# TankMermaid/GraphAligner

Measured on AMD Instinct MI355X. Metric: aligned Gbp/sec (whole node), 10kb ONT reads vs chr-scale GFA, higher is better.
Workload: dtype u64

## Files before the change

graphaligner_amd/csrc/ga_device.hip:

```cpp
#include <hip/hip_runtime.h>

#include <algorithm>
#include <cstdio>
#include <cstdlib>
#include <cstring>
#include <memory>
#include <mutex>
#include <vector>

#include "../../include/graphaligner_amd.h"
#include "ga_backend.h"
#include "ga_kernel.h"
#include "ga_lanes.h"
#include "ga_seed_dev.h"

namespace {

#define HIP_OK(call) do { hipError_t e_ = (call); if (e_ != hipSuccess) { fprintf(stderr, "graphaligner_amd: %s failed: %s\n", #call, hipGetErrorString(e_)); return GA_E_DEVICE; } } while (0)

struct SlotLayout
{
	uint64_t endPrev, endCur, sliceOff, arena, trace, flags, ckpt, belowOff, sparse, ovr, bytes;
};
__host__ __device__ inline SlotLayout slotLayout(uint32_t capCols, uint32_t maxSlices, uint64_t arenaWords, uint32_t traceCap, uint32_t sparseBw = 0)
{
	auto up = [](uint64_t x) { return (x + 255) & ~255ull; };
	SlotLayout l;
	uint64_t at = 0;
	l.endPrev = at; at = up(at + 4ull * capCols);
	l.endCur = at; at = up(at + 4ull * capCols);
	l.sliceOff = at; at = up(at + 4ull * (maxSlices + 1));
	l.arena = at; at = up(at + 4ull * arenaWords);
	l.trace = at; at = up(at + 1ull * traceCap + 64);
	l.flags = at; at = up(at + maxSlices + 1);
	l.ckpt = at; at = up(at + 4ull * (maxSlices + 2));
	l.belowOff = at; at = up(at + 4ull * (maxSlices + 1));
	l.sparse = at; if (sparseBw) at = up(at + gak::sparse_mem_bytes(sparseBw));
	l.ovr = at; if (sparseBw) at = up(at + 8ull * (maxSlices + 2));
	l.bytes = at;
	return l;
}

#ifndef GA_WAVES_EU
#define GA_WAVES_EU 4
#endif
template <int MAXN, bool GENERAL, bool SPARSE = false>
__global__ void __launch_bounds__(64) __attribute__((amdgpu_waves_per_eu(GA_WAVES_EU, 8))) ga_extend_kernel(GaLaunch L)
{
	__shared__ gak::WaveState<MAXN> ws;
	const SlotLayout lay = slotLayout(L.cap_cols, L.max_slices, L.arena_words, L.trace_cap, SPARSE ? L.sparse_bw : 0u);
	uint8_t* base = L.scratch + (uint64_t)blockIdx.x * L.slot_bytes;
	gak::Slot slot;
	slot.end_prev = (uint32_t*)(base + lay.endPrev);
	slot.end_cur = (uint32_t*)(base + lay.endCur);
	slot.slice_off = (uint32_t*)(base + lay.sliceOff);
	slot.arena = (uint32_t*)(base + lay.arena);
	slot.trace = base + lay.trace;
	slot.slice_flags = base + lay.flags;
	slot.ckpt = (uint32_t*)(base + lay.ckpt);
	slot.below_off = (uint32_t*)(base + lay.belowOff);
	slot.sparse = SPARSE ? base + lay.sparse : nullptr;
	slot.ovr = SPARSE ? (uint32_t*)(base + lay.ovr) : nullptr;
	slot.sparse_max_bw = SPARSE ? L.sparse_bw : 0u;
	while (true)
	{
		uint32_t k = gaw::wave_atomic_add(L.next_job, 1u);
		if (k >= L.n_jobs) break;
		uint32_t job = L.job_list ? L.job_list[k] : k;
		gak::run_job<MAXN, GENERAL, SPARSE>(L, ws, slot, job);
		__syncthreads();
	}
}

template <int N, int LW>
__global__ void __launch_bounds__(64) __attribute__((amdgpu_waves_per_eu(1, 2))) ga_lanes_kernel(gal::GaLanesLaunch L)
{
	using namespace gal;
	__shared__ uint32_t lds[Lay<N>::WORDS * LW + LW * kStageWords64 * 2 + 128];
	const int lane = (int)threadIdx.x;
	const WaveLayout lay = wave_layout<N>(L.cap_cols, L.cap_rows, L.max_slices, L.cap_moves, LW);
	uint8_t* base = L.scratch + (uint64_t)blockIdx.x * L.wave_bytes;
	while (true)
	{
		const uint32_t grp = gaw::wave_atomic_add(L.next_group, 1u);
		const uint64_t first = (uint64_t)grp * L.lanes_per_wave;
		if (first >= L.n_jobs) break;
		const bool hasJob = lane < (int)L.lanes_per_wave && lane < LW && first + (uint32_t)lane < L.n_jobs;
		const uint32_t jobIndex = hasJob ? (L.job_list ? L.job_list[first + (uint32_t)lane] : (uint32_t)(first + (uint32_t)lane)) : 0u;
		LaneMem m;
		m.lane = lane < LW ? lane : 0;
		m.tid = lane;
		m.flushPart = (uint32_t)lane % 12u; m.flushLane = (uint32_t)lane / 12u;
		m.ls = LW;
		m.lds.base = lds + (lane < LW ? lane : 0);
		m.lds.lw = LW;
		m.stage = (uint64_t*)(lds + Lay<N>::WORDS * LW);
		m.laneBlocks = lds + Lay<N>::WORDS * LW + LW * kStageWords64 * 2;
		m.usedChunks = 12u * (L.lanes_per_wave < (uint32_t)LW ? L.lanes_per_wave : (uint32_t)LW);
		m.endPrev = (uint32_t*)(base + lay.endA) + m.lane;
		m.endCur = (uint32_t*)(base + lay.endB) + m.lane;
		m.hdr = (uint32_t*)(base + lay.hdr) + m.lane;
		m.snodes = (uint32_t*)(base + lay.snodes) + m.lane;
		m.moves = (uint32_t*)(base + lay.moves) + m.lane;
		m.arena = base + lay.arena;
		LaneState st;
#if GA_STAMPS == 3
		const uint64_t wall0 = wall_clock64(), cyc0 = gaw::stamp();
#endif
		uint64_t tA = gaw::stamp(), tB, acc[4] = {0, 0, 0, 0};
#define GAL_LAP(i) do { tB = gaw::stamp(); acc[i] += tB - tA; tA = tB; } while (0)
		lane_begin<N>(L, m, st, jobIndex, hasJob);
		uint32_t blockTop = 0;
		for (uint32_t slice = 0; ; slice++)
		{
			lane_band<N>(L, m, st, slice);
			GAL_LAP(0);
			if (!__ballot(st.live)) break;
			fill_slice<N, 8, LW>(L.graph, m, st, slice, st.live, blockTop, L.cap_rows, L.cap_cols);
			GAL_LAP(1);
			lane_end_slice<N>(L, m, st, slice);
			GAL_LAP(2);
		}
		lane_finish<N>(L, m, st, hasJob);
		GAL_LAP(3);
#undef GAL_LAP
#ifdef GA_STAMPS
		if (hasJob && lane == 0) { GaJobOut* o = L.outs + st.job; o->stamps[1] = acc[0]; o->stamps[4] = acc[1]; o->stamps[0] = acc[2]; o->stamps[5] = acc[3]; o->stamps[2] = st.laps[0]; o->stamps[3] = st.laps[1]; o->stamps[6] = st.laps[2]; o->stamps[7] = st.laps[7];
#if GA_STAMPS == 4
			o->stamps[6] = acc[0]; o->stamps[7] = acc[1];
			for (int i = 0; i < 5; i++) o->stamps[i] = st.blaps[i];
#endif
#if GA_STAMPS == 3
			o->stamps[0] = wall0; o->stamps[1] = wall_clock64(); o->stamps[4] = gaw::stamp() - cyc0;
#endif
#if GA_STAMPS == 2
			o->stamps[0] = st.laps[4]; o->stamps[1] = st.laps[5]; o->stamps[4] = st.laps[6];
#endif
		}
#endif
		__syncthreads();
	}
}

__global__ void __launch_bounds__(64) ga_eq_words_kernel(const uint8_t* __restrict__ seq, const GaEqFill* __restrict__ fills, uint32_t nFills, const uint8_t* __restrict__ lut,
                                                         uint32_t padCode, uint64_t* __restrict__ eq, uint8_t* __restrict__ flags, uint8_t* __restrict__ rows)
{
	__shared__ uint8_t t[512];
	const uint32_t lane = threadIdx.x;
	for (uint32_t i = lane; i < 512; i += 64) t[i] = lut[i];
	__syncthreads();
	for (uint32_t fi = blockIdx.x; fi < nFills; fi += gridDim.x)
	{
		const GaEqFill f = fills[fi];
		const uint8_t* s = seq + f.seq_off;
		bool bad = false;
		for (uint32_t r0 = 0; r0 < f.padded; r0 += 64)
		{
			const uint32_t k = r0 + lane;
			uint32_t code = padCode;
			if (k < f.n) code = f.backward ? t[256 + s[f.n - 1 - k]] : t[s[f.pos + k]];
			rows[f.eq_slice * 64 + k] = (uint8_t)code;
			const uint64_t e0 = __ballot(code & 1u), e1 = __ballot(code & 2u), e2 = __ballot(code & 4u), e3 = __ballot(code & 8u);
			const uint64_t inv = __ballot(code & GA_ROW_INVALID);
			const uint32_t last = (uint32_t)__builtin_amdgcn_readlane((int)code, 63);
			const uint64_t meta = (uint64_t)((last >> 4) & 7u) | (inv ? 8u : 0u);
			if (lane < 5) eq[(f.eq_slice + r0 / 64) * 5 + lane] = lane == 0 ? e0 : lane == 1 ? e1 : lane == 2 ? e2 : lane == 3 ? e3 : meta;
			bad = bad || inv != 0;
		}
		if (lane == 0) flags[fi] = bad ? 1 : 0;
	}
}

__global__ void ga_outs_init_kernel(GaJobOut* outs, uint32_t n)
{
	const uint32_t i = blockIdx.x * blockDim.x + threadIdx.x;
	if (i >= n) return;
	GaJobOut o;
	memset(&o, 0, sizeof(o));
	o.status = GA_NOT_RUN;
	outs[i] = o;
}

struct PinnedPool
{
	std::mutex lock;
	std::vector<std::pair<size_t, char*>> idle;
	~PinnedPool() { for (auto& b : idle) hipHostFree(b.second); }
};

struct DevGraph : GaBackendGraph
{
	std::shared_ptr<PinnedPool> pinned = std::make_shared<PinnedPool>();
	bool buildsMatchWords() const override { return true; }
	std::shared_ptr<char> hostBlock(size_t bytes) override
	{
		const size_t two = (size_t)2 << 20;
		bytes = (bytes + two - 1) & ~(two - 1);
		std::shared_ptr<PinnedPool> pool = pinned;
		char* p = nullptr;
		size_t cap = 0;
		{
			std::lock_guard<std::mutex> guard(pool->lock);
			size_t best = pool->idle.size();
			for (size_t i = 0; i < pool->idle.size(); i++)
				if (pool->idle[i].first >= bytes && pool->idle[i].first <= 2 * bytes + two && (best == pool->idle.size() || pool->idle[i].first < pool->idle[best].first)) best = i;
			if (best != pool->idle.size()) { cap = pool->idle[best].first; p = pool->idle[best].second; pool->idle.erase(pool->idle.begin() + (long)best); }
		}
		if (!p)
		{
			hipSetDevice(device);
			if (hipHostMalloc((void**)&p, bytes, hipHostMallocDefault) != hipSuccess) return GaBackendGraph::hostBlock(bytes);
			cap = bytes;
		}
		return std::shared_ptr<char>(p, [pool, cap](char* q) {
			std::lock_guard<std::mutex> guard(pool->lock);
			if (pool->idle.size() < 6) pool->idle.emplace_back(cap, q); else hipHostFree(q);
		});
	}

	std::unique_ptr<gasd::DevSeedEngine> seed;
	GaSeedEngine* seedEngine() override { return seed.get(); }

	int device = 0;
	GaDevGraph g;
	GaHmmTables* hmm = nullptr;
	std::vector<void*> allocs;
	int cus = 0;
	uint64_t totalBp = 0;
	uint8_t* pool = nullptr;
	size_t poolBytes = 0;
	bool poolBusy = false;
	~DevGraph() override
	{
		hipSetDevice(device);
		for (void* p : allocs) hipFree(p);
		for (auto& b : idleBlocks) hipFree(b.second);
		if (pool) hipFree(pool);
		if (hostPool) hipHostFree(hostPool);
	}
	std::mutex blockLock;
	std::vector<std::pair<size_t, void*>> idleBlocks;
	void* takeBlock(size_t bytes)
	{
		{
			std::lock_guard<std::mutex> lock(blockLock);
			size_t best = idleBlocks.size();
			for (size_t i = 0; i < idleBlocks.size(); i++)
				if (idleBlocks[i].first >= bytes && idleBlocks[i].first <= bytes + bytes / 2 + 4096 && (best == idleBlocks.size() || idleBlocks[i].first < idleBlocks[best].first)) best = i;
			if (best != idleBlocks.size())
			{
				void* p = idleBlocks[best].second;
				idleBlocks.erase(idleBlocks.begin() + (long)best);
				return p;
			}
		}
		void* p = nullptr;
		if (hipMalloc(&p, bytes) != hipSuccess) return nullptr;
		return p;
	}
	void giveBlock(void* p, size_t bytes)
	{
		std::lock_guard<std::mutex> lock(blockLock);
		if (idleBlocks.size() >= 48) { hipFree(idleBlocks.front().second); idleBlocks.erase(idleBlocks.begin()); }
		idleBlocks.emplace_back(bytes, p);
	}
	std::mutex poolLock;
	uint8_t* takePool(size_t bytes)
	{
		std::lock_guard<std::mutex> lock(poolLock);
		if (poolBusy) return nullptr;
		if (bytes > poolBytes)
		{
			if (pool) hipFree(pool);
			pool = nullptr; poolBytes = 0;
			if (hipMalloc((void**)&pool, bytes) != hipSuccess) { pool = nullptr; return nullptr; }
			poolBytes = bytes;
		}
		poolBusy = true;
		return pool;
	}
	void givePool() { std::lock_guard<std::mutex> lock(poolLock); poolBusy = false; }
	size_t poolBytesIfFree() { std::lock_guard<std::mutex> lock(poolLock); return poolBusy ? 0 : poolBytes; }
	std::mutex hostLock;
	uint8_t* hostPool = nullptr;
	size_t hostPoolBytes = 0;
	bool hostPoolBusy = false;
	uint8_t* takeHost(size_t bytes)
	{
		std::lock_guard<std::mutex> lock(hostLock);
		if (hostPoolBusy) return nullptr;
		if (bytes > hostPoolBytes)
		{
			if (hostPool) hipHostFree(hostPool);
			hostPool = nullptr; hostPoolBytes = 0;
			const size_t want = bytes + bytes / 8;
			if (hipHostMalloc((void**)&hostPool, want, hipHostMallocDefault) != hipSuccess) { hostPool = nullptr; return nullptr; }
			hostPoolBytes = want;
		}
		hostPoolBusy = true;
		return hostPool;
	}
	void giveHost() { std::lock_guard<std::mutex> lock(hostLock); hostPoolBusy = false; }
	template <typename T> int put(const std::vector<T>& v, const T** out)
	{
		void* p = nullptr;
		HIP_OK(hipMalloc(&p, std::max<size_t>(v.size() * sizeof(T), 16)));
		allocs.push_back(p);
		HIP_OK(hipMemcpy(p, v.data(), v.size() * sizeof(T), hipMemcpyHostToDevice));
		*out = (const T*)p;
		return 0;
	}
};

struct Knobs
{
	int lanes = -1;
	int spread = 1;
	bool debugPasses = false;
	uint64_t tracePoolBytes = 0;
	Knobs()
	{
		if (const char* e = getenv("GA_LANES")) lanes = atoi(e) != 0 ? 1 : 0;
		debugPasses = getenv("GA_DEBUG_PASSES") != nullptr;
		if (const char* e = getenv("GA_LANES_SPREAD")) spread = atoi(e);
		if (const char* t = getenv("GA_TEST_TRACE_POOL_BYTES")) tracePoolBytes = (uint64_t)atoll(t) & ~3ull;
	}
};

struct DevBatch : GaBackendBatch
{
	DevGraph* g = nullptr;
	Knobs knobs;
	hipStream_t stream = nullptr;
	hipEvent_t evA = nullptr, evB = nullptr;
	std::vector<std::pair<size_t, void*>> allocs;
	std::vector<GaJob> jobs;
	GaRunConfig cfg;
	GaLaunch L;
	const uint64_t* dEq = nullptr;
	uint32_t* dList = nullptr;
	size_t dListCap = 0;
	std::vector<GaJobOut> outs;
	bool outsLocked = false;
	std::vector<uint32_t> orderHost;
	std::vector<uint8_t> passOf;
	int passNo = 0;
	GaRunStats st;
	GaRowsProvider rowsProvider;
	uint8_t* privateScratch = nullptr;
	size_t privateBytes = 0;

	~DevBatch() override
	{
		hipSetDevice(g->device);
		if (hostFromPool) g->giveHost();
		if (outsLocked) hipHostUnregister(outs.data());
		for (auto& a : allocs) g->giveBlock(a.second, a.first);
		if (privateScratch) hipFree(privateScratch);
		if (evA) hipEventDestroy(evA);
		if (evB) hipEventDestroy(evB);
		if (stream) hipStreamDestroy(stream);
	}
	template <typename T> int alloc(T** out, size_t count)
	{
		const size_t bytes = (std::max<size_t>(count * sizeof(T), 16) + 255) & ~(size_t)255;
		void* p = g->takeBlock(bytes);
		if (!p) { fprintf(stderr, "graphaligner_amd: no device memory for %zu bytes\n", bytes); return GA_E_DEVICE; }
		allocs.emplace_back(bytes, p);
		*out = (T*)p;
		return 0;
	}

	int ensureRows()
	{
		if (L.rows) return 0;
		if (builtRows) { L.rows = builtRows; return 0; }
		const std::vector<uint8_t>& rows = rowsProvider();
		uint8_t* dRows;
		if (alloc(&dRows, rows.size())) return GA_E_DEVICE;
		HIP_OK(hipMemcpyAsync(dRows, rows.data(), rows.size(), hipMemcpyHostToDevice, stream));
		L.rows = dRows;
		return 0;
	}

	uint8_t* builtRows = nullptr;
	std::vector<uint8_t> badFills;
	const std::vector<uint8_t>* invalidFills() const override { return &badFills; }
	bool emittingRuns() const override { return cfg.emit_runs != 0; }

	int init(const uint64_t* eq, const GaEqSource* src, size_t eqWords, const std::vector<GaJob>& jobsIn)
	{
		HIP_OK(hipSetDevice(g->device));
		HIP_OK(hipStreamCreateWithFlags(&stream, hipStreamNonBlocking));
		HIP_OK(hipEventCreate(&evA));
		HIP_OK(hipEventCreate(&evB));
		jobs = jobsIn;
		memset(&L, 0, sizeof(L));
		L.graph = g->g;
		L.hmm = g->hmm;
		L.n_jobs = (uint32_t)jobs.size();
		L.initial_bw = cfg.initial_bw;
		L.ramp_bw = cfg.ramp_bw;
		L.max_slices = std::max<uint32_t>(cfg.max_slices, 1);
		GaJob* dJobs; uint64_t* eqDev;
		if (alloc(&eqDev, eqWords)) return GA_E_DEVICE;
		if (alloc(&dJobs, jobs.size())) return GA_E_DEVICE;
		if (!src && !eq) return GA_E_INVALID;
		if (src)
		{
			uint8_t *dSeq, *dLut, *dFlags, *dRows; GaEqFill* dFills;
			const size_t rowBytes = (eqWords / 5) * 64 + 64;
			if (alloc(&dSeq, src->seqBytes + 64) || alloc(&dFills, src->nFills) || alloc(&dLut, 512) || alloc(&dFlags, src->nFills) || alloc(&dRows, rowBytes)) return GA_E_DEVICE;
			HIP_OK(hipMemsetAsync(dRows + rowBytes - 128, 0, 128, stream));
			builtRows = dRows;
			uint8_t lut[512];
			memcpy(lut, src->rowCode, 256); memcpy(lut + 256, src->rowCodeRc, 256);
			HIP_OK(hipMemcpyAsync(dSeq, src->seq, src->seqBytes, hipMemcpyHostToDevice, stream));
			HIP_OK(hipMemcpyAsync(dFills, src->fills, src->nFills * sizeof(GaEqFill), hipMemcpyHostToDevice, stream));
			HIP_OK(hipMemcpyAsync(dLut, lut, 512, hipMemcpyHostToDevice, stream));
			HIP_OK(hipMemsetAsync(eqDev + (eqWords - 5), 0, 40, stream));
			badFills.assign(src->nFills, 0);
			if (src->nFills)
			{
				const uint32_t blocks = (uint32_t)std::min<size_t>(src->nFills, (size_t)g->cus * 64);
				hipLaunchKernelGGL(ga_eq_words_kernel, dim3(blocks), dim3(64), 0, stream, dSeq, dFills, (uint32_t)src->nFills, dLut, (uint32_t)src->padCode, eqDev, dFlags, dRows);
				HIP_OK(hipGetLastError());
				HIP_OK(hipMemcpyAsync(badFills.data(), dFlags, src->nFills, hipMemcpyDeviceToHost, stream));
			}
			HIP_OK(hipStreamSynchronize(stream));
			for (uint8_t f : badFills) if (f) { cfg.emit_runs = 0; break; }
		}
		else HIP_OK(hipMemcpyAsync(eqDev, eq, eqWords * 8, hipMemcpyHostToDevice, stream));
		HIP_OK(hipMemcpyAsync(dJobs, jobs.data(), jobs.size() * sizeof(GaJob), hipMemcpyHostToDevice, stream));
		L.rows = nullptr;
		L.jobs = dJobs;
		dEq = eqDev;
		orderHost.resize(jobs.size());
		for (uint32_t i = 0; i < jobs.size(); i++) orderHost[i] = i;
		std::stable_sort(orderHost.begin(), orderHost.end(), [&](uint32_t a, uint32_t b) { return jobs[a].n_rows > jobs[b].n_rows; });
		dListCap = std::max<size_t>(jobs.size(), 1);
		if (alloc(&dList, dListCap)) return GA_E_DEVICE;
		if (alloc(&L.outs, jobs.size())) return GA_E_DEVICE;
		outs.assign(jobs.size(), GaJobOut{});
		for (auto& o : outs) o.status = GA_NOT_RUN;
		outsLocked = !outs.empty() && hipHostRegister(outs.data(), outs.size() * sizeof(GaJobOut), hipHostRegisterDefault) == hipSuccess;
		if (alloc(&L.next_job, 4)) return GA_E_DEVICE;
		if (alloc(&L.trace_top, 2)) return GA_E_DEVICE;
		uint64_t totalRows = 0;
		for (auto& j : jobs) totalRows += j.n_rows;
		L.trace_pool_cap = ((totalRows * (cfg.emit_runs ? 4 : 1) + totalRows / 2 + 256ull * jobs.size() + 4096) + 3) & ~3ull;
		if (knobs.tracePoolBytes) L.trace_pool_cap = knobs.tracePoolBytes;
		if (alloc(&L.traces, L.trace_pool_cap)) return GA_E_DEVICE;
		HIP_OK(hipStreamSynchronize(stream));
		return 0;
	}

	uint8_t* takeScratch(size_t bytes, bool& fromPool)
	{
		uint8_t* p = g->takePool(bytes);
		fromPool = p != nullptr;
		if (p) return p;
		if (bytes > privateBytes)
		{
			if (privateScratch) hipFree(privateScratch);
			privateScratch = nullptr; privateBytes = 0;
			if (hipMalloc((void**)&privateScratch, bytes) != hipSuccess) { privateScratch = nullptr; return nullptr; }
			privateBytes = bytes;
		}
		return privateScratch;
	}
	size_t scratchBudget() const
	{
		size_t freeB = 0, totalB = 0;
		if (hipMemGetInfo(&freeB, &totalB) != hipSuccess) return 0;
		const size_t poolFree = g->poolBytesIfFree();
		return (size_t)((freeB + (poolFree ? poolFree : privateBytes)) * 0.85);
	}
	int uploadList(const std::vector<uint32_t>& list)
	{
		HIP_OK(hipMemcpyAsync(dList, list.data(), list.size() * 4, hipMemcpyHostToDevice, stream));
		return 0;
	}
	int afterPass(float& ms)
	{
		HIP_OK(hipGetLastError());
		HIP_OK(hipEventRecord(evB, stream));
		HIP_OK(hipMemcpyAsync(outs.data(), L.outs, outs.size() * sizeof(GaJobOut), hipMemcpyDeviceToHost, stream));
		HIP_OK(hipStreamSynchronize(stream));
		HIP_OK(hipEventElapsedTime(&ms, evA, evB));
		st.kernel_ms += ms;
		return 0;
	}

	static bool isCapacity(int s) { return s == GA_CAP_NODES || s == GA_CAP_COLS || s == GA_CAP_ARENA || s == GA_CAP_TRACE || s == GA_CAP_HEAP || s == GA_PUNT || s == GA_NOT_RUN; }
	static bool needsGeneral(int s) { return s == GA_UNSUPPORTED_CYCLE || s == GA_UNSUPPORTED_RAMP; }
	static bool widerLanes(int s) { return s == GA_CAP_NODES || s == GA_CAP_COLS || s == GA_CAP_ARENA || s == GA_CAP_TRACE || s == GA_CAP_HEAP; }

	template <int N, int LW> int lanesPass(const std::vector<uint32_t>& list, uint32_t rowsPerSlice, bool first)
	{
		if (list.empty()) return 0;
		for (uint32_t i : list) passOf[i] = (uint8_t)passNo;
		passNo++;
		gal::GaLanesLaunch P;
		memset(&P, 0, sizeof(P));
		P.graph = L.graph; P.hmm = L.hmm; P.eq = dEq; P.jobs = L.jobs; P.outs = L.outs;
		P.job_list = dList; P.n_jobs = (uint32_t)list.size();
		P.lanes_per_wave = LW;
		P.next_group = L.next_job;
		P.traces = L.traces; P.trace_top = L.trace_top; P.trace_pool_cap = L.trace_pool_cap;
		P.initial_bw = L.initial_bw; P.ramp_bw = L.ramp_bw;
		P.emit_runs = cfg.emit_runs;
		uint32_t maxRows = 0;
		for (uint32_t i : list) maxRows = std::max(maxRows, jobs[i].n_rows);
		P.max_slices = std::max<uint32_t>(maxRows / 64, 1);
		P.cap_cols = std::min<uint32_t>(N * 256u, 0xff00u);
		P.cap_moves = maxRows * 2 + 1024;
		const uint32_t ldsBytes = gal::Lay<N>::WORDS * LW * 4 + LW * gal::kStageWords64 * 8 + 512;
		const uint32_t wavesPerCu = std::max<uint32_t>(1, std::min<uint32_t>(8, 163840u / ldsBytes));
		auto layoutFor = [&](uint32_t lanes) {
			P.cap_rows = (uint32_t)std::min<uint64_t>(((uint64_t)P.max_slices * rowsPerSlice * lanes + 64 + 7u) & ~7ull, 0x7ffffff0ull);
			return gal::wave_layout<N>(P.cap_cols, P.cap_rows, P.max_slices, P.cap_moves, LW);
		};
		gal::WaveLayout lay = layoutFor(LW);
		const uint64_t fit = scratchBudget() / std::max<uint64_t>(lay.bytes, 1);
		const uint64_t slotsHere = std::max<uint64_t>(1, std::min<uint64_t>((uint64_t)g->cus * wavesPerCu, std::max<uint64_t>(fit, 64)));
		uint32_t lanesPer = LW;
		if (knobs.spread > 1) lanesPer = (uint32_t)std::min<int>(LW, knobs.spread);
		else if (knobs.spread && list.size() * 10 < slotsHere * LW * 6)
			lanesPer = (uint32_t)std::min<uint64_t>(LW, std::max<uint64_t>(8, (list.size() + slotsHere - 1) / slotsHere));
		P.lanes_per_wave = lanesPer;
		lay = layoutFor(lanesPer);
		P.wave_bytes = lay.bytes;
		const uint64_t groups = (list.size() + lanesPer - 1) / lanesPer;
		const uint32_t waves = (uint32_t)std::max<uint64_t>(1, std::min<uint64_t>(slotsHere, groups));
		bool fromPool = false;
		uint8_t* scratch = takeScratch((size_t)waves * lay.bytes, fromPool);
		if (!scratch) return 0;
		P.scratch = scratch;
		int rc = uploadList(list);
		if (!rc)
		{
			hipMemsetAsync(L.next_job, 0, 16, stream);
			hipEventRecord(evA, stream);
			hipLaunchKernelGGL((ga_lanes_kernel<N, LW>), dim3(waves), dim3(64), 0, stream, P);
			float ms = 0;
			rc = afterPass(ms);
			if (first) { st.main_ms = ms; st.main_variant = N * 1000 + 80 + (LW == 64 ? 0 : 1); st.slots = waves; st.waves_per_cu = wavesPerCu; st.scratch_bytes = (uint64_t)waves * lay.bytes; }
			if (knobs.debugPasses) fprintf(stderr, "graphaligner_amd: lanes pass <%d,%d>: %zu jobs on %u waves (%.1f GB scratch), %.2f ms\n", N, LW, list.size(), waves, waves * (double)lay.bytes / 1e9, ms);
#if GA_STAMPS == 3
			{
				uint64_t lo = ~0ull, hi = 0, n = 0; double life = 0, cyc = 0, lateStart = 0;
				for (auto& o : outs) if (o.stamps[1]) { lo = std::min(lo, o.stamps[0]); hi = std::max(hi, o.stamps[1]); }
				for (auto& o : outs) if (o.stamps[1]) { n++; life += (double)(o.stamps[1] - o.stamps[0]); cyc += (double)o.stamps[4]; lateStart = std::max(lateStart, (double)(o.stamps[0] - lo)); }
				{
					std::vector<std::pair<double, uint64_t>> lives;
					for (auto& o : outs) if (o.stamps[1]) lives.push_back({(double)(o.stamps[1] - o.stamps[0]) / 1e5, o.stamps[7]});
					std::sort(lives.begin(), lives.end());
					auto at = [&](double q) { return lives[(size_t)(q * (lives.size() - 1))]; };
					if (!lives.empty()) fprintf(stderr, "graphaligner_amd: wave life ms p10 %.2f p50 %.2f p90 %.2f p99 %.2f max %.2f; traceback rounds of the p10 / p50 / p99 / max wave: %llu / %llu / %llu / %llu, fast iterations %llu / %llu / %llu / %llu\n",
						at(0.1).first, at(0.5).first, at(0.9).first, at(0.99).first, at(1.0).first,
						(unsigned long long)(at(0.1).second & 0xffffffffu), (unsigned long long)(at(0.5).second & 0xffffffffu), (unsigned long long)(at(0.99).second & 0xffffffffu), (unsigned long long)(at(1.0).second & 0xffffffffu),
						(unsigned long long)(at(0.1).second >> 32), (unsigned long long)(at(0.5).second >> 32), (unsigned long long)(at(0.99).second >> 32), (unsigned long long)(at(1.0).second >> 32));
				}
				if (n) fprintf(stderr, "graphaligner_amd: %llu waves: first start to last end %.3f ms, mean wave life %.3f ms = %.1f M shader cycles (%.2f GHz), latest start %.3f ms after the first\n",
				               (unsigned long long)n, (hi - lo) / 1e5, life / n / 1e5, cyc / n / 1e6, cyc / life / 10.0, lateStart / 1e5);
			}
#endif
		}
		if (fromPool) g->givePool();
		return rc;
	}

	template <int MAXN, bool GENERAL, bool SPARSE = false> int retryPass(uint32_t capCols, uint64_t arenaWordsPerSlice, uint32_t traceMul, uint32_t wavesPerCuRetry, bool takeCapacity, bool takeGeneral,
	                                                                    uint64_t arenaWordsExtra = 0)
	{
		std::vector<uint32_t> again;
		for (uint32_t i : orderHost)
			if ((takeCapacity && isCapacity(outs[i].status)) || (takeGeneral && needsGeneral(outs[i].status)) || (SPARSE && outs[i].status == GA_UNSUPPORTED_BAND)) again.push_back(i);
		if (again.empty()) return 0;
		if (ensureRows()) return GA_E_DEVICE;
		for (uint32_t i : again) passOf[i] = (uint8_t)passNo;
		passNo++;
		st.jobs_retried += again.size();
		GaLaunch Rl = L;
		uint32_t maxRows = 0;
		for (uint32_t i : again) maxRows = std::max(maxRows, jobs[i].n_rows);
		Rl.cap_cols = capCols;
		Rl.trace_cap = maxRows * traceMul + 4096;
		Rl.max_slices = std::max<uint32_t>(maxRows / 64, 1);
		Rl.arena_words = std::min<uint64_t>(64 + (uint64_t)(maxRows / 64) * (gak::kSliceHdrWords + arenaWordsPerSlice) + arenaWordsExtra, 0xfffffff0ull);
		Rl.sparse_bw = SPARSE ? (uint32_t)std::max(std::max(L.initial_bw, L.ramp_bw), 1) : 0u;
		SlotLayout lay = slotLayout(Rl.cap_cols, Rl.max_slices, Rl.arena_words, Rl.trace_cap, Rl.sparse_bw);
		Rl.slot_bytes = lay.bytes;
		const uint64_t fit = scratchBudget() / lay.bytes;
		uint32_t rslots = (uint32_t)std::max<uint64_t>(1, std::min<uint64_t>(std::min<uint64_t>((uint64_t)g->cus * wavesPerCuRetry, fit), again.size()));
		bool fromPool = false;
		uint8_t* scratch = takeScratch((size_t)rslots * lay.bytes, fromPool);
		if (!scratch) return 0;
		Rl.scratch = scratch;
		if (passNo == 1) { st.slots = rslots; st.waves_per_cu = wavesPerCuRetry; st.scratch_bytes = (uint64_t)rslots * lay.bytes; }
		Rl.job_list = dList;
		Rl.n_jobs = (uint32_t)again.size();
		int rc = uploadList(again);
		if (!rc)
		{
			hipMemsetAsync(Rl.next_job, 0, 16, stream);
			if (SPARSE) hipMemset2DAsync(scratch + lay.sparse, lay.bytes, 0, gak::sparse_mem_bytes(Rl.sparse_bw), rslots, stream);
			hipEventRecord(evA, stream);
			hipLaunchKernelGGL((ga_extend_kernel<MAXN, GENERAL, SPARSE>), dim3(rslots), dim3(64), 0, stream, Rl);
			float ms = 0;
			rc = afterPass(ms);
			if (knobs.debugPasses) fprintf(stderr, "graphaligner_amd: wave-per-read pass <%d,%d>: %zu jobs on %u slots, %.2f ms\n", MAXN, (int)GENERAL, again.size(), rslots, ms);
		}
		if (fromPool) g->givePool();
		return rc;
	}

	int run() override
	{
		HIP_OK(hipSetDevice(g->device));
		st = GaRunStats();
		passOf.assign(jobs.size(), 0);
		passNo = 0;
		if (jobs.empty()) return 0;
		for (auto& o : outs) o.status = GA_NOT_RUN;
		hipLaunchKernelGGL(ga_outs_init_kernel, dim3((uint32_t)((jobs.size() + 255) / 256)), dim3(256), 0, stream, L.outs, (uint32_t)jobs.size());
		HIP_OK(hipGetLastError());
		HIP_OK(hipMemsetAsync(L.trace_top, 0, 16, stream));
		const double meanNode = g->g.n_nodes > 2 ? (double)g->totalBp / (double)(g->g.n_nodes - 2) : 64.0;
		const bool useLanes = knobs.lanes >= 0 ? knobs.lanes != 0 : meanNode >= 40;
		int rc = 0;
		if (useLanes)
		{
			const int startN = meanNode >= 40 ? 0 : meanNode >= 14 ? 1 : 2;
			std::vector<uint32_t> list = orderHost;
			bool first = true;
			for (int n = startN; n <= 2 && !list.empty() && !rc; n++)
			{
				if (!first && list.size() < 512) break;
				if (n == 0) rc = lanesPass<10, 64>(list, 288, first);
				else if (n == 1) rc = lanesPass<24, 32>(list, 480, first);
				else rc = lanesPass<56, 16>(list, 768, first);
				first = false;
				std::vector<uint32_t> again;
				for (uint32_t i : list) if (widerLanes(outs[i].status)) again.push_back(i);
				list.swap(again);
			}
			if (rc) return rc;
		}
		st.jobs_retried = 0;
		if (!useLanes)
		{
#ifndef GA_FIRST_N
#define GA_FIRST_N 32
#endif
			rc = retryPass<GA_FIRST_N, false>(4096, 3 * 64 + 5 * 800, 2, 24, true, false);
			if (rc) return rc;
			st.main_ms = st.kernel_ms;
			st.main_variant = -GA_FIRST_N;
			st.jobs_retried = 0;
		}
		rc = retryPass<64, false>(8192, 3 * 64 + 5 * 2048, 3, 12, true, false);
		if (rc) return rc;
		rc = retryPass<64, true>(8192, 3 * 64 + 5 * 4096, 4, 8, false, true);
		if (rc) return rc;
		rc = retryPass<256, true>(65536, 3 * 256 + 5 * 8192, 6, 4, true, true);
		if (rc) return rc;
		rc = retryPass<256, true, true>(1u << 20, 3 * 256 + 5 * 20000, 8, 1, true, true, 48ull << 20);
		for (int k = 0; k < 8; k++) { st.stamps[k] = 0; for (auto& o : outs) st.stamps[k] += o.stamps[k]; }
		return rc;
	}

	uint8_t* hostTraces = nullptr;
	bool hostFromPool = false;
	std::unique_ptr<uint8_t[]> hostPrivate;
	size_t hostPrivateBytes = 0;
	int fetch(std::vector<GaJobOut>& o, const uint8_t** traces, uint64_t* nBytes) override
	{
		HIP_OK(hipSetDevice(g->device));
		fetchDone();
		o = outs;
		for (size_t i = 0; i < o.size(); i++) o[i].reserved2 = passOf[i];
		uint64_t top = 0;
		HIP_OK(hipMemcpyAsync(&top, L.trace_top, 8, hipMemcpyDeviceToHost, stream));
		HIP_OK(hipStreamSynchronize(stream));
		top = std::min<uint64_t>(top, L.trace_pool_cap);
		hostTraces = g->takeHost(top + 64);
		hostFromPool = hostTraces != nullptr;
		if (!hostTraces)
		{
			if (hostPrivateBytes < top + 64) { hostPrivate.reset(new uint8_t[top + 64]); hostPrivateBytes = top + 64; }
			hostTraces = hostPrivate.get();
		}
		if (top)
		{
			HIP_OK(hipMemcpyAsync(hostTraces, L.traces, top, hipMemcpyDeviceToHost, stream));
			HIP_OK(hipStreamSynchronize(stream));
		}
		*traces = hostTraces;
		*nBytes = top;
		return 0;
	}
	void fetchDone() override
	{
		if (hostFromPool) g->giveHost();
		hostFromPool = false;
		hostTraces = nullptr;
	}
	GaRunStats stats() const override { return st; }
};

}

GaBackendGraph* ga_backend_upload_graph(const GaFlatGraph& flat, const GaHmmTables& hmm, int device, int* status)
{
	int count = 0;
	if (hipGetDeviceCount(&count) != hipSuccess || count <= 0 || device < 0 || device >= count) { *status = GA_E_NO_DEVICE; return nullptr; }
	if (hipSetDevice(device) != hipSuccess) { *status = GA_E_NO_DEVICE; return nullptr; }
	hipDeviceProp_t prop;
	if (hipGetDeviceProperties(&prop, device) != hipSuccess) { *status = GA_E_NO_DEVICE; return nullptr; }
	if (flat.node_start.size() - 1 >= 0xfffffff0ull) { *status = GA_E_INVALID; return nullptr; }
	DevGraph* g = new DevGraph();
	g->device = device;
	g->cus = prop.multiProcessorCount;
	g->g.n_nodes = (uint32_t)(flat.node_start.size() - 1);
	g->g.reserved = 0;
	g->totalBp = flat.node_start.back();
	int bad = 0;
	bad |= g->put(flat.node_start, &g->g.node_start);
	bad |= g->put(flat.seq2, &g->g.seq2);
	bad |= g->put(flat.in_off, &g->g.in_off);
	bad |= g->put(flat.in_nbr, &g->g.in_nbr);
	bad |= g->put(flat.out_off, &g->g.out_off);
	bad |= g->put(flat.out_nbr, &g->g.out_nbr);
	bad |= g->put(ga_build_node_records(flat), &g->g.node_rec);
	std::vector<GaHmmTables> h(1, hmm);
	const GaHmmTables* dh = nullptr;
	bad |= g->put(h, &dh);
	g->hmm = const_cast<GaHmmTables*>(dh);
	if (bad) { delete g; *status = GA_E_DEVICE; return nullptr; }
	g->seed = std::make_unique<gasd::DevSeedEngine>(g, device, g->cus, g->g);
	*status = 0;
	return g;
}

GaBackendBatch* ga_backend_create_batch(GaBackendGraph* graph, GaRowsProvider rows, const uint64_t* eq, const GaEqSource* src, size_t eqWords, const std::vector<GaJob>& jobs,
                                        const GaRunConfig& cfg, int* status)
{
	DevBatch* b = new DevBatch();
	b->g = static_cast<DevGraph*>(graph);
	b->cfg = cfg;
	b->rowsProvider = rows;
	int s = b->init(eq, src, eqWords, jobs);
	if (s) { delete b; *status = s; return nullptr; }
	*status = 0;
	return b;
}
```

Before: 15.54.

## Copy back a byte status plane per pass instead of full job outputs

After each pass a small kernel gathers each job's status into a byte array, and only that array is copied to the host. The full GaJobOut array is now copied once, in fetch. A histogram of present statuses lets passes with nothing to retry skip building their lists, and the first lanes pass reads a pre-uploaded order list. The counter and trace-top resets are folded into the init kernel, and scratch is taken from an already-held pool without re-deriving the budget. Risks: correctness depends on hStatus staying in sync, maxRows now assumes lists are sorted by row count, and fetch adds one large synchronous copy.

Result: slower. 9.519 (-38.7%).

```diff
diff --git a/graphaligner_amd/csrc/ga_device.hip b/graphaligner_amd/csrc/ga_device.hip
--- a/graphaligner_amd/csrc/ga_device.hip
+++ b/graphaligner_amd/csrc/ga_device.hip
@@ -1,11 +1,13 @@
 #include <hip/hip_runtime.h>
 
 #include <algorithm>
+#include <chrono>
 #include <cstdio>
 #include <cstdlib>
 #include <cstring>
 #include <memory>
 #include <mutex>
+#include <string>
 #include <vector>
 
 #include "../../include/graphaligner_amd.h"
@@ -171,14 +173,24 @@
 	}
 }
 
-__global__ void ga_outs_init_kernel(GaJobOut* outs, uint32_t n)
+__global__ void ga_outs_init_kernel(GaJobOut* outs, uint8_t* plane, uint32_t n, uint32_t* nextJob, uint64_t* traceTop)
 {
 	const uint32_t i = blockIdx.x * blockDim.x + threadIdx.x;
+	if (i < 4) nextJob[i] = 0;
+	if (i < 2) traceTop[i] = 0;
 	if (i >= n) return;
 	GaJobOut o;
 	memset(&o, 0, sizeof(o));
 	o.status = GA_NOT_RUN;
 	outs[i] = o;
+	plane[i] = (uint8_t)GA_NOT_RUN;
+}
+
+constexpr uint32_t kGatherBlock = 256;
+__global__ void __launch_bounds__(kGatherBlock) ga_status_gather_kernel(const GaJobOut* __restrict__ outs, uint8_t* __restrict__ plane, uint32_t n)
+{
+	const uint32_t i = blockIdx.x * kGatherBlock + threadIdx.x;
+	if (i < n) plane[i] = (uint8_t)outs[i].status;
 }
 
 struct PinnedPool
@@ -279,6 +291,13 @@
 		poolBusy = true;
 		return pool;
 	}
+	uint8_t* takePoolIfHeld(size_t bytes)
+	{
+		std::lock_guard<std::mutex> lock(poolLock);
+		if (poolBusy || bytes > poolBytes) return nullptr;
+		poolBusy = true;
+		return pool;
+	}
 	void givePool() { std::lock_guard<std::mutex> lock(poolLock); poolBusy = false; }
 	size_t poolBytesIfFree() { std::lock_guard<std::mutex> lock(poolLock); return poolBusy ? 0 : poolBytes; }
 	std::mutex hostLock;
@@ -317,11 +336,13 @@
 	int lanes = -1;
 	int spread = 1;
 	bool debugPasses = false;
+	bool waitEvent = false;
 	uint64_t tracePoolBytes = 0;
 	Knobs()
 	{
 		if (const char* e = getenv("GA_LANES")) lanes = atoi(e) != 0 ? 1 : 0;
 		debugPasses = getenv("GA_DEBUG_PASSES") != nullptr;
+		if (const char* e = getenv("GA_RUN_WAIT_EVENT")) waitEvent = atoi(e) != 0;
 		if (const char* e = getenv("GA_LANES_SPREAD")) spread = atoi(e);
 		if (const char* t = getenv("GA_TEST_TRACE_POOL_BYTES")) tracePoolBytes = (uint64_t)atoll(t) & ~3ull;
 	}
@@ -332,7 +353,7 @@
 	DevGraph* g = nullptr;
 	Knobs knobs;
 	hipStream_t stream = nullptr;
-	hipEvent_t evA = nullptr, evB = nullptr;
+	hipEvent_t evA = nullptr, evB = nullptr, evDone = nullptr;
 	std::vector<std::pair<size_t, void*>> allocs;
 	std::vector<GaJob> jobs;
 	GaRunConfig cfg;
@@ -340,12 +361,25 @@
 	const uint64_t* dEq = nullptr;
 	uint32_t* dList = nullptr;
 	size_t dListCap = 0;
+	uint32_t* dOrder = nullptr;
+	uint8_t* dStatus = nullptr;
+	std::vector<uint8_t> statusHost;
+	uint8_t* hStatus = nullptr;
+	bool statusLocked = false;
+	bool present[256] = {};
+	bool queueZeroed = false;
 	std::vector<GaJobOut> outs;
 	bool outsLocked = false;
 	std::vector<uint32_t> orderHost;
 	std::vector<uint8_t> passOf;
 	int passNo = 0;
 	GaRunStats st;
+	typedef std::chrono::steady_clock Clock;
+	Clock::time_point runT0;
+	double lapLaunch = -1;
+	std::vector<double> lapAfter;
+	static double msSince(Clock::time_point t) { return std::chrono::duration<double, std::milli>(Clock::now() - t).count(); }
+	void lapLaunched() { if (lapLaunch < 0) lapLaunch = msSince(runT0); }
 	GaRowsProvider rowsProvider;
 	uint8_t* privateScratch = nullptr;
 	size_t privateBytes = 0;
@@ -355,10 +389,12 @@
 		hipSetDevice(g->device);
 		if (hostFromPool) g->giveHost();
 		if (outsLocked) hipHostUnregister(outs.data());
+		if (statusLocked) hipHostUnregister(hStatus);
 		for (auto& a : allocs) g->giveBlock(a.second, a.first);
 		if (privateScratch) hipFree(privateScratch);
 		if (evA) hipEventDestroy(evA);
 		if (evB) hipEventDestroy(evB);
+		if (evDone) hipEventDestroy(evDone);
 		if (stream) hipStreamDestroy(stream);
 	}
 	template <typename T> int alloc(T** out, size_t count)
@@ -394,6 +430,7 @@
 		HIP_OK(hipStreamCreateWithFlags(&stream, hipStreamNonBlocking));
 		HIP_OK(hipEventCreate(&evA));
 		HIP_OK(hipEventCreate(&evB));
+		HIP_OK(hipEventCreateWithFlags(&evDone, hipEventBlockingSync | hipEventDisableTiming));
 		jobs = jobsIn;
 		memset(&L, 0, sizeof(L));
 		L.graph = g->g;
@@ -440,7 +477,13 @@
 		std::stable_sort(orderHost.begin(), orderHost.end(), [&](uint32_t a, uint32_t b) { return jobs[a].n_rows > jobs[b].n_rows; });
 		dListCap = std::max<size_t>(jobs.size(), 1);
 		if (alloc(&dList, dListCap)) return GA_E_DEVICE;
+		if (alloc(&dOrder, dListCap)) return GA_E_DEVICE;
+		HIP_OK(hipMemcpyAsync(dOrder, orderHost.data(), orderHost.size() * 4, hipMemcpyHostToDevice, stream));
 		if (alloc(&L.outs, jobs.size())) return GA_E_DEVICE;
+		if (alloc(&dStatus, jobs.size())) return GA_E_DEVICE;
+		statusHost.assign(std::max<size_t>(jobs.size(), 16), (uint8_t)GA_NOT_RUN);
+		hStatus = statusHost.data();
+		statusLocked = hipHostRegister(hStatus, statusHost.size(), hipHostRegisterDefault) == hipSuccess;
 		outs.assign(jobs.size(), GaJobOut{});
 		for (auto& o : outs) o.status = GA_NOT_RUN;
 		outsLocked = !outs.empty() && hipHostRegister(outs.data(), outs.size() * sizeof(GaJobOut), hipHostRegisterDefault) == hipSuccess;
@@ -481,14 +524,43 @@
 		HIP_OK(hipMemcpyAsync(dList, list.data(), list.size() * 4, hipMemcpyHostToDevice, stream));
 		return 0;
 	}
+	void scanPlane()
+	{
+		memset(present, 0, sizeof(present));
+		const size_t n = jobs.size();
+		size_t i = 0;
+		for (; i + 8 <= n; i += 8)
+		{
+			uint64_t w;
+			memcpy(&w, hStatus + i, 8);
+			if (!w) { present[0] = true; continue; }
+			for (size_t k = i; k < i + 8; k++) present[hStatus[k]] = true;
+		}
+		for (; i < n; i++) present[hStatus[i]] = true;
+	}
 	int afterPass(float& ms)
 	{
+		const Clock::time_point t0 = Clock::now();
+		lapLaunched();
 		HIP_OK(hipGetLastError());
 		HIP_OK(hipEventRecord(evB, stream));
+		const uint32_t n = (uint32_t)jobs.size();
+		hipLaunchKernelGGL(ga_status_gather_kernel, dim3((n + kGatherBlock - 1) / kGatherBlock), dim3(kGatherBlock), 0, stream, L.outs, dStatus, n);
+		HIP_OK(hipGetLastError());
+		HIP_OK(hipMemcpyAsync(hStatus, dStatus, n, hipMemcpyDeviceToHost, stream));
+#if GA_STAMPS
 		HIP_OK(hipMemcpyAsync(outs.data(), L.outs, outs.size() * sizeof(GaJobOut), hipMemcpyDeviceToHost, stream));
-		HIP_OK(hipStreamSynchronize(stream));
+#endif
+		if (knobs.waitEvent)
+		{
+			HIP_OK(hipEventRecord(evDone, stream));
+			HIP_OK(hipEventSynchronize(evDone));
+		}
+		else HIP_OK(hipStreamSynchronize(stream));
+		scanPlane();
 		HIP_OK(hipEventElapsedTime(&ms, evA, evB));
 		st.kernel_ms += ms;
+		lapAfter.push_back(msSince(t0));
 		return 0;
 	}
 
@@ -499,19 +571,19 @@
 	template <int N, int LW> int lanesPass(const std::vector<uint32_t>& list, uint32_t rowsPerSlice, bool first)
 	{
 		if (list.empty()) return 0;
-		for (uint32_t i : list) passOf[i] = (uint8_t)passNo;
+		const bool whole = &list == &orderHost;
+		if (passNo) for (uint32_t i : list) passOf[i] = (uint8_t)passNo;
 		passNo++;
 		gal::GaLanesLaunch P;
 		memset(&P, 0, sizeof(P));
 		P.graph = L.graph; P.hmm = L.hmm; P.eq = dEq; P.jobs = L.jobs; P.outs = L.outs;
-		P.job_list = dList; P.n_jobs = (uint32_t)list.size();
+		P.job_list = whole ? dOrder : dList; P.n_jobs = (uint32_t)list.size();
 		P.lanes_per_wave = LW;
 		P.next_group = L.next_job;
 		P.traces = L.traces; P.trace_top = L.trace_top; P.trace_pool_cap = L.trace_pool_cap;
 		P.initial_bw = L.initial_bw; P.ramp_bw = L.ramp_bw;
 		P.emit_runs = cfg.emit_runs;
-		uint32_t maxRows = 0;
-		for (uint32_t i : list) maxRows = std::max(maxRows, jobs[i].n_rows);
+		const uint32_t maxRows = jobs[list.front()].n_rows;
 		P.max_slices = std::max<uint32_t>(maxRows / 64, 1);
 		P.cap_cols = std::min<uint32_t>(N * 256u, 0xff00u);
 		P.cap_moves = maxRows * 2 + 1024;
@@ -521,26 +593,42 @@
 			P.cap_rows = (uint32_t)std::min<uint64_t>(((uint64_t)P.max_slices * rowsPerSlice * lanes + 64 + 7u) & ~7ull, 0x7ffffff0ull);
 			return gal::wave_layout<N>(P.cap_cols, P.cap_rows, P.max_slices, P.cap_moves, LW);
 		};
-		gal::WaveLayout lay = layoutFor(LW);
-		const uint64_t fit = scratchBudget() / std::max<uint64_t>(lay.bytes, 1);
-		const uint64_t slotsHere = std::max<uint64_t>(1, std::min<uint64_t>((uint64_t)g->cus * wavesPerCu, std::max<uint64_t>(fit, 64)));
-		uint32_t lanesPer = LW;
-		if (knobs.spread > 1) lanesPer = (uint32_t)std::min<int>(LW, knobs.spread);
-		else if (knobs.spread && list.size() * 10 < slotsHere * LW * 6)
-			lanesPer = (uint32_t)std::min<uint64_t>(LW, std::max<uint64_t>(8, (list.size() + slotsHere - 1) / slotsHere));
-		P.lanes_per_wave = lanesPer;
-		lay = layoutFor(lanesPer);
-		P.wave_bytes = lay.bytes;
-		const uint64_t groups = (list.size() + lanesPer - 1) / lanesPer;
-		const uint32_t waves = (uint32_t)std::max<uint64_t>(1, std::min<uint64_t>(slotsHere, groups));
-		bool fromPool = false;
-		uint8_t* scratch = takeScratch((size_t)waves * lay.bytes, fromPool);
+		gal::WaveLayout lay;
+		uint32_t lanesPer = LW, waves = 0;
+		auto plan = [&](uint64_t slotsHere) {
+			lanesPer = LW;
+			if (knobs.spread > 1) lanesPer = (uint32_t)std::min<int>(LW, knobs.spread);
+			else if (knobs.spread && list.size() * 10 < slotsHere * LW * 6)
+				lanesPer = (uint32_t)std::min<uint64_t>(LW, std::max<uint64_t>(8, (list.size() + slotsHere - 1) / slotsHere));
+			P.lanes_per_wave = lanesPer;
+			lay = layoutFor(lanesPer);
+			P.wave_bytes = lay.bytes;
+			const uint64_t groups = (list.size() + lanesPer - 1) / lanesPer;
+			waves = (uint32_t)std::max<uint64_t>(1, std::min<uint64_t>(slotsHere, groups));
+		};
+		plan((uint64_t)g->cus * wavesPerCu);
+		bool fromPool = true;
+		uint8_t* scratch = g->takePoolIfHeld((size_t)waves * lay.bytes);
+		if (!scratch)
+		{
+			const uint64_t budget = scratchBudget();
+			const uint64_t fit = budget / std::max<uint64_t>(layoutFor(LW).bytes, 1);
+			plan(std::max<uint64_t>(1, std::min<uint64_t>((uint64_t)g->cus * wavesPerCu, std::max<uint64_t>(fit, 64))));
+			waves = (uint32_t)std::min<uint64_t>(waves, budget / std::max<uint64_t>(lay.bytes, 1));
+			if (!waves)
+			{
+				if (knobs.debugPasses) fprintf(stderr, "graphaligner_amd: lanes pass <%d,%d>: %zu jobs skipped, no room for one wave (%.3f GB) in a budget of %.3f GB\n", N, LW, list.size(), lay.bytes / 1e9, budget / 1e9);
+				return 0;
+			}
+			scratch = takeScratch((size_t)waves * lay.bytes, fromPool);
+		}
 		if (!scratch) return 0;
 		P.scratch = scratch;
-		int rc = uploadList(list);
+		int rc = whole ? 0 : uploadList(list);
 		if (!rc)
 		{
-			hipMemsetAsync(L.next_job, 0, 16, stream);
+			if (!queueZeroed) hipMemsetAsync(L.next_job, 0, 16, stream);
+			queueZeroed = false;
 			hipEventRecord(evA, stream);
 			hipLaunchKernelGGL((ga_lanes_kernel<N, LW>), dim3(waves), dim3(64), 0, stream, P);
 			float ms = 0;
@@ -574,17 +662,19 @@
 	template <int MAXN, bool GENERAL, bool SPARSE = false> int retryPass(uint32_t capCols, uint64_t arenaWordsPerSlice, uint32_t traceMul, uint32_t wavesPerCuRetry, bool takeCapacity, bool takeGeneral,
 	                                                                    uint64_t arenaWordsExtra = 0)
 	{
+		bool take[256];
+		for (int s = 0; s < 256; s++) take[s] = (takeCapacity && isCapacity(s)) || (takeGeneral && needsGeneral(s)) || (SPARSE && s == GA_UNSUPPORTED_BAND);
+		bool any = false;
+		for (int s = 0; s < 256; s++) any = any || (take[s] && present[s]);
+		if (!any) return 0;
 		std::vector<uint32_t> again;
-		for (uint32_t i : orderHost)
-			if ((takeCapacity && isCapacity(outs[i].status)) || (takeGeneral && needsGeneral(outs[i].status)) || (SPARSE && outs[i].status == GA_UNSUPPORTED_BAND)) again.push_back(i);
-		if (again.empty()) return 0;
+		for (uint32_t i : orderHost) if (take[hStatus[i]]) again.push_back(i);
 		if (ensureRows()) return GA_E_DEVICE;
-		for (uint32_t i : again) passOf[i] = (uint8_t)passNo;
+		if (passNo) for (uint32_t i : again) passOf[i] = (uint8_t)passNo;
 		passNo++;
 		st.jobs_retried += again.size();
 		GaLaunch Rl = L;
-		uint32_t maxRows = 0;
-		for (uint32_t i : again) maxRows = std::max(maxRows, jobs[i].n_rows);
+		const uint32_t maxRows = jobs[again.front()].n_rows;
 		Rl.cap_cols = capCols;
 		Rl.trace_cap = maxRows * traceMul + 4096;
 		Rl.max_slices = std::max<uint32_t>(maxRows / 64, 1);
@@ -592,10 +682,15 @@
 		Rl.sparse_bw = SPARSE ? (uint32_t)std::max(std::max(L.initial_bw, L.ramp_bw), 1) : 0u;
 		SlotLayout lay = slotLayout(Rl.cap_cols, Rl.max_slices, Rl.arena_words, Rl.trace_cap, Rl.sparse_bw);
 		Rl.slot_bytes = lay.bytes;
-		const uint64_t fit = scratchBudget() / lay.bytes;
-		uint32_t rslots = (uint32_t)std::max<uint64_t>(1, std::min<uint64_t>(std::min<uint64_t>((uint64_t)g->cus * wavesPerCuRetry, fit), again.size()));
-		bool fromPool = false;
-		uint8_t* scratch = takeScratch((size_t)rslots * lay.bytes, fromPool);
+		uint32_t rslots = (uint32_t)std::max<uint64_t>(1, std::min<uint64_t>((uint64_t)g->cus * wavesPerCuRetry, again.size()));
+		bool fromPool = true;
+		uint8_t* scratch = g->takePoolIfHeld((size_t)rslots * lay.bytes);
+		if (!scratch)
+		{
+			const uint64_t fit = scratchBudget() / lay.bytes;
+			rslots = (uint32_t)std::max<uint64_t>(1, std::min<uint64_t>(std::min<uint64_t>((uint64_t)g->cus * wavesPerCuRetry, fit), again.size()));
+			scratch = takeScratch((size_t)rslots * lay.bytes, fromPool);
+		}
 		if (!scratch) return 0;
 		Rl.scratch = scratch;
 		if (passNo == 1) { st.slots = rslots; st.waves_per_cu = wavesPerCuRetry; st.scratch_bytes = (uint64_t)rslots * lay.bytes; }
@@ -604,7 +699,8 @@
 		int rc = uploadList(again);
 		if (!rc)
 		{
-			hipMemsetAsync(Rl.next_job, 0, 16, stream);
+			if (!queueZeroed) hipMemsetAsync(Rl.next_job, 0, 16, stream);
+			queueZeroed = false;
 			if (SPARSE) hipMemset2DAsync(scratch + lay.sparse, lay.bytes, 0, gak::sparse_mem_bytes(Rl.sparse_bw), rslots, stream);
 			hipEventRecord(evA, stream);
 			hipLaunchKernelGGL((ga_extend_kernel<MAXN, GENERAL, SPARSE>), dim3(rslots), dim3(64), 0, stream, Rl);
@@ -618,33 +714,57 @@
 
 	int run() override
 	{
+		runT0 = Clock::now();
+		lapLaunch = -1;
+		lapAfter.clear();
+		const int rc = runPasses();
+		if (knobs.debugPasses)
+		{
+			const double wall = msSince(runT0);
+			double waits = 0;
+			std::string each;
+			for (double a : lapAfter) { waits += a; char buf[32]; snprintf(buf, sizeof(buf), "%s%.3f", each.empty() ? "" : " ", a); each += buf; }
+			const double launch = lapLaunch < 0 ? 0 : lapLaunch;
+			fprintf(stderr, "graphaligner_amd: run: wall %.3f ms = to first launch %.3f + after-pass [%s] %.3f + other host %.3f; kernels %.3f ms, wall - kernels %.3f, after-pass - kernels %.3f\n",
+			        wall, launch, each.c_str(), waits, wall - launch - waits, st.kernel_ms, wall - st.kernel_ms, waits - st.kernel_ms);
+		}
+		return rc;
+	}
+	int runPasses()
+	{
 		HIP_OK(hipSetDevice(g->device));
 		st = GaRunStats();
 		passOf.assign(jobs.size(), 0);
 		passNo = 0;
 		if (jobs.empty()) return 0;
-		for (auto& o : outs) o.status = GA_NOT_RUN;
-		hipLaunchKernelGGL(ga_outs_init_kernel, dim3((uint32_t)((jobs.size() + 255) / 256)), dim3(256), 0, stream, L.outs, (uint32_t)jobs.size());
+		memset(hStatus, GA_NOT_RUN, jobs.size());
+		memset(present, 0, sizeof(present));
+		present[GA_NOT_RUN] = true;
+		hipLaunchKernelGGL(ga_outs_init_kernel, dim3((uint32_t)((jobs.size() + 255) / 256)), dim3(256), 0, stream, L.outs, dStatus, (uint32_t)jobs.size(), L.next_job, L.trace_top);
 		HIP_OK(hipGetLastError());
-		HIP_OK(hipMemsetAsync(L.trace_top, 0, 16, stream));
+		queueZeroed = true;
 		const double meanNode = g->g.n_nodes > 2 ? (double)g->totalBp / (double)(g->g.n_nodes - 2) : 64.0;
 		const bool useLanes = knobs.lanes >= 0 ? knobs.lanes != 0 : meanNode >= 40;
 		int rc = 0;
 		if (useLanes)
 		{
 			const int startN = meanNode >= 40 ? 0 : meanNode >= 14 ? 1 : 2;
-			std::vector<uint32_t> list = orderHost;
+			std::vector<uint32_t> rest;
 			bool first = true;
-			for (int n = startN; n <= 2 && !list.empty() && !rc; n++)
+			for (int n = startN; n <= 2 && !rc; n++)
 			{
+				const std::vector<uint32_t>& list = first ? orderHost : rest;
+				if (list.empty()) break;
 				if (!first && list.size() < 512) break;
 				if (n == 0) rc = lanesPass<10, 64>(list, 288, first);
 				else if (n == 1) rc = lanesPass<24, 32>(list, 480, first);
 				else rc = lanesPass<56, 16>(list, 768, first);
+				bool any = false;
+				for (int s = 0; s < 256; s++) any = any || (present[s] && widerLanes(s));
+				std::vector<uint32_t> again;
+				if (any) for (uint32_t i : list) if (widerLanes(hStatus[i])) again.push_back(i);
 				first = false;
-				std::vector<uint32_t> again;
-				for (uint32_t i : list) if (widerLanes(outs[i].status)) again.push_back(i);
-				list.swap(again);
+				rest.swap(again);
 			}
 			if (rc) return rc;
 		}
@@ -667,7 +787,9 @@
 		rc = retryPass<256, true>(65536, 3 * 256 + 5 * 8192, 6, 4, true, true);
 		if (rc) return rc;
 		rc = retryPass<256, true, true>(1u << 20, 3 * 256 + 5 * 20000, 8, 1, true, true, 48ull << 20);
+#if GA_STAMPS
 		for (int k = 0; k < 8; k++) { st.stamps[k] = 0; for (auto& o : outs) st.stamps[k] += o.stamps[k]; }
+#endif
 		return rc;
 	}
 
@@ -679,6 +801,11 @@
 	{
 		HIP_OK(hipSetDevice(g->device));
 		fetchDone();
+		if (!outs.empty())
+		{
+			HIP_OK(hipMemcpyAsync(outs.data(), L.outs, outs.size() * sizeof(GaJobOut), hipMemcpyDeviceToHost, stream));
+			HIP_OK(hipStreamSynchronize(stream));
+		}
 		o = outs;
 		for (size_t i = 0; i < o.size(); i++) o[i].reserved2 = passOf[i];
 		uint64_t top = 0;
```
